# chahuja/mix-stage

Measured on AMD Instinct MI355X. Metric: train-step clips/sec (B=32, T=64, M=8), higher is better.
Workload: dtype f32; 1 GPU; Mix-StAGE GAN train step (reference D/G coin flip, seed 4321: 457 G + 510 D steps), B=32 clips per GPU, T=64, 128-mel, 104-dim pose, M=S=8, audio branch pinned; fp32 arithmetic (the reference trains in fp64, trainer.py:138; held to it at 1e-4 pose L1); global_batch=32, parallelism=dp1, hip_graphs=True, bn_sync=local

## Files before the change

### include/mixstage_aux.h

```cpp
#ifndef MIXSTAGE_AUX_H_
#define MIXSTAGE_AUX_H_

#include "mixstage.h"

#ifdef __cplusplus
extern "C" {
#endif

int ms_set_counter_buffer(int32_t* zeroed_counters, int n);

int ms_conv_block_bwd_overlap(const ms_conv_desc* d, const float* x, const float* x2, const float* w,
                              const float* gamma, const float* running_mean, const float* running_var,
                              const float* y_raw, const float* y, const float* save, const float* dy, float* dyr,
                              float* dx, float* dx2, float* dw, float* dbias, float* dgamma, float* dbeta,
                              void* workspace, size_t workspace_bytes, void* stream, void* side_stream,
                              void* side_workspace, size_t side_workspace_bytes);

int ms_timing_enable(int on);
size_t ms_timing_report(char* buf, size_t cap);

int ms_debug_set_patch_min_workgroups(int n);
int ms_debug_set_patch_tuning(int intra_split, int force_splitk);

int ms_debug_set_conv16_tile(int wm, int wn);
int ms_debug_set_conv16_ring(int nstg, int wide8);
int ms_debug_set_wgrad16_target(int workgroups);
int ms_debug_set_wgrad16_ring(int buffers);
int ms_debug_set_wgrad_target(int workgroups);
int ms_debug_set_wgrad_wave(int on);
int ms_debug_set_conv_tile(int on);
int ms_debug_set_bn_fused(int on);
int ms_debug_set_bn_fused_min_workgroups(int n);
int ms_debug_set_skip(const char* patterns);

int ms_debug_set_clip32(int on);

int ms_debug_set_clip_corun(int on);
int ms_debug_set_clip_corun_bwd(int on);

int ms_selftest_mfma(const float* A, const float* B, float* C, int K, void* stream);
int ms_probe_peak(int kind, long iters, void* a, void* b, double* work, void* stream);

#ifdef __cplusplus
}
#endif
#endif
```

### mix_stage_amd/_lib.py

```python
import ctypes
import os

_HERE = os.path.dirname(os.path.abspath(__file__))
LIB_PATH = os.path.join(_HERE, 'libmixstage_hip.so')
_ALT_LIB = os.environ.get('MS_LIB_PATH')
if _ALT_LIB:
  LIB_PATH = _ALT_LIB

c_void_p, c_int, c_float, c_size_t = ctypes.c_void_p, ctypes.c_int, ctypes.c_float, ctypes.c_size_t


class BwdOptions(ctypes.Structure):
  _fields_ = [('side_stream', ctypes.c_void_p), ('side_workspace', ctypes.c_void_p), ('side_workspace_bytes', ctypes.c_size_t),
              ('wt_prepared', ctypes.c_void_p), ('wgrad_partials', ctypes.c_void_p), ('defer_wgrad_launch', ctypes.c_int),
              ('prev_y', ctypes.c_void_p), ('prev_y_raw', ctypes.c_void_p), ('prev_save', ctypes.c_void_p), ('prev_gamma', ctypes.c_void_p),
              ('prev_dgamma', ctypes.c_void_p), ('prev_dbeta', ctypes.c_void_p), ('prev_dbias', ctypes.c_void_p), ('prev_slope', ctypes.c_float),
              ('bn_sync', ctypes.c_void_p), ('bn_sync_words', ctypes.c_int32), ('dy_is_dyr', ctypes.c_int),
              ('dx_accum', ctypes.c_void_p)]


class LossScale(ctypes.Structure):
  _fields_ = [('scale', ctypes.c_float), ('scale_dev', ctypes.c_void_p)]


# ... 126 lines not shown
    'ms_debug_set_patch_min_workgroups': (c_int, [c_int]),
    'ms_debug_set_patch_tuning': (c_int, [c_int, c_int]),
    'ms_debug_set_conv16_tile': (c_int, [c_int, c_int]),
    'ms_debug_set_conv16_ring': (c_int, [c_int, c_int]),
    'ms_debug_set_skip': (c_int, [ctypes.c_char_p]),
    'ms_debug_set_clip32': (c_int, [c_int]),
    'ms_debug_set_clip_corun': (c_int, [c_int]),
    'ms_clip_hold': (c_int, [_P]),
    'ms_clip_hold_flush': (c_int, [_P]),
    'ms_clip_hold_discard': (c_int, [_P]),
    'ms_clip_grid': (c_int, [_DESC]),
    'ms_clip_pair_ok': (c_int, [_DESC, _DESC]),
    'ms_clip_dgrad_grid': (c_int, [_DESC]),
    'ms_clip_dgrad_pair_ok': (c_int, [_DESC, _DESC]),
    'ms_debug_set_clip_corun_bwd': (c_int, [c_int]),
    'ms_debug_set_wgrad16_target': (c_int, [c_int]),
    'ms_debug_set_wgrad16_ring': (c_int, [c_int]),
    'ms_debug_set_wgrad_target': (c_int, [c_int]),
    'ms_debug_set_wgrad_wave': (c_int, [c_int]),
    'ms_debug_set_conv_tile': (c_int, [c_int]),
    'ms_set_wgrad_batched': (c_int, [c_int, c_int]),
    'ms_dgrad_fuses_prev_bn': (c_int, [_P]),
    'ms_dgrad_takes_accum': (c_int, [_P]),
    'ms_stat_pair_ok': (c_int, [_P]),
    'ms_selftest_mfma': (c_int, [_P, _P, _P, c_int, _P]),
    'ms_probe_peak': (c_int, [c_int, ctypes.c_long, _P, _P, ctypes.POINTER(ctypes.c_double), _P]),
}

_lib = None

# ... 17 lines not shown
    mode = os.environ.get('MS_PRECISION', '')
    if mode:
      if mode not in ('fp32', 'bf16x6'):
        raise MixStageLibError('MS_PRECISION=%s: expected fp32 or bf16x6' % mode)
      handle.ms_set_precision(1 if mode == 'bf16x6' else 0)
    if os.environ.get('MS_BN_FUSED'):
      handle.ms_debug_set_bn_fused(int(os.environ['MS_BN_FUSED']))
    if os.environ.get('MS_BN_FUSED_MIN_WGS'):
      handle.ms_debug_set_bn_fused_min_workgroups(int(os.environ['MS_BN_FUSED_MIN_WGS']))
    if os.environ.get('MS_CLIP32'):
      handle.ms_debug_set_clip32(int(os.environ['MS_CLIP32']))
    if os.environ.get('MS_CONV_TILE'):
      handle.ms_debug_set_conv_tile(int(os.environ['MS_CONV_TILE']))
    if os.environ.get('MS_WGRAD_WAVE'):
      handle.ms_debug_set_wgrad_wave(int(os.environ['MS_WGRAD_WAVE']))
    if os.environ.get('MS_PATCH_MIN_WGS'):
      handle.ms_debug_set_patch_min_workgroups(int(os.environ['MS_PATCH_MIN_WGS']))
    _lib = handle
  return _lib


def check(rc, what):
  if rc != 0:
    raise MixStageLibError('%s failed: %s' % (what, lib().ms_last_error().decode()))
```

### mix_stage_amd/csrc/api.hip

```cpp
#include "block_geom.h"

namespace ms {
extern int g_clip32;

static int validate(const ms_conv_desc* d, const char* who) {
  if (!d) return set_error("%s: null descriptor", who);
  if (d->B < 1 || d->Cin < 1 || d->Cout < 1 || d->groups < 1 || d->H < 1 || d->W < 1 || d->KH < 1 || d->KW < 1 ||
      d->SH < 1 || d->SW < 1 || d->PH < 0 || d->PW < 0)
    return set_error("%s: bad geometry", who);
  const int oh = (d->H + 2 * d->PH - d->KH) / d->SH + 1, ow = (d->W + 2 * d->PW - d->KW) / d->SW + 1;
  if (d->H + 2 * d->PH < d->KH || d->W + 2 * d->PW < d->KW || oh != d->OH || ow != d->OW)
    return set_error("%s: output size (%d,%d) does not match geometry (expected %d,%d)", who, d->OH, d->OW, oh, ow);
  if (d->mode < MS_BARE || d->mode > MS_BN_EVAL) return set_error("%s: bad mode %d", who, d->mode);
  if (d->in_mode < MS_IN_PLAIN || d->in_mode > MS_IN_UP2ADD) return set_error("%s: bad in_mode %d", who, d->in_mode);
  if (d->in_mode == MS_IN_UP2ADD && (d->H != 1 || d->KH != 1 || (d->W & 1)))
    return set_error("%s: UP2ADD needs a 1-D block with even W", who);
  if (dt_of(d) > DT_F16 || (d->dtype & ~(0xff | MS_DT_OUT_F32 | MS_DT_BN_FOLDED | MS_DT_STAT_PAIR))) return set_error("%s: bad dtype 0x%x", who, d->dtype);
  if (dt_of(d) == DT_F32 && (d->dtype & ~(0xff | MS_DT_STAT_PAIR))) return set_error("%s: MS_DT_OUT_F32 is a flag of the 16-bit modes", who);
  if ((d->dtype & MS_DT_STAT_PAIR) && (d->B & 1)) return set_error("%s: MS_DT_STAT_PAIR needs an even batch", who);
  const double out_elems = (double)d->B * d->groups * d->Cout * d->OH * d->OW;
  const double in_elems = (double)d->B * d->groups * d->Cin * d->H * d->W;
  const double lim = dt_of(d) == DT_F32 ? 536870912.0 : 1073741824.0;
  if (out_elems >= lim || in_elems >= lim) return set_error("%s: tensor of 2 GiB or more (%.0f elements)", who, std::max(out_elems, in_elems));
  return 0;
// ... 513 lines not shown
  float* colpart = ws_at<float>(workspace, p.ws.colpart);
  float* wt = ws_at<float>(workspace, p.ws.wt);
  float* wg_part = ws_at<float>(workspace, p.ws.wg_part);
  float* dg_part = ws_at<float>(workspace, p.ws.dg_part);
  if (defer_wgrad) wg_part = opt->wgrad_partials;
  hipStream_t ws_stream = s;
  if (side_stream && side_stream != stream && dw) {
    if (defer_wgrad) return set_error("ms_conv_block_bwd_ex: wgrad_partials and side_stream are exclusive");
    if (!opt->side_workspace || opt->side_workspace_bytes < p.ws.total)
      return set_error("ms_conv_block_bwd_overlap: side workspace too small");
    ws_stream = (hipStream_t)side_stream;
    wg_part = ws_at<float>(opt->side_workspace, p.ws.wg_part);
  }

  const float* gr = dy;
  int bias_done = 0;
  const bool have_prev = opt->prev_y != nullptr;
  if (have_prev && !(dx && g_precision == 0 && clip32_dgrad_bn_ok(d)))
    return set_error("ms_conv_block_bwd: this block's data gradient cannot carry the producer's BatchNorm backward (ms_dgrad_fuses_prev_bn)");
  if (opt->dy_is_dyr) {
    if (d->mode != MS_BN_TRAIN) return set_error("ms_conv_block_bwd: dy_is_dyr is the BN_TRAIN form");
    bias_done = 1;
  } else if (d->mode == MS_BN_TRAIN) {
    rc = launch_bn_bwd(dy, y_raw, y, save, gamma, bn_part, dyr, colpart, dbias, dgamma, dbeta, d->B, C, hw, d->slope, &bias_done, s, sg_of(d));
    gr = dyr;
  } else if (d->mode == MS_LRELU) {
    rc = launch_act_bwd(dy, y, dyr, colpart, dbias, d->B, C, hw, 1, d->slope, &bias_done, s);
    gr = dyr;
  } else if (dbias) {
    rc = launch_act_bwd(dy, nullptr, nullptr, colpart, dbias, d->B, C, hw, 0, 0.f, &bias_done, s);
  }
  if (rc) return rc;
  if (dbias && !bias_done && !opt->dy_is_dyr) {
    rc = launch_colsum_finalize(colpart, dbias, d->B, C, s);
    if (rc) return rc;
  }

  if (ws_stream != s) {
    hipEvent_t ev = fork_event();
// ... 99 lines not shown
      if (pl.splitk > 1) {
        a.part = dg_part;
        a.part_stride = dx_elems;
        a.ep = EP_DGRAD;
      }
      rc = launch_gather(a, true, up2, pl, s);
      if (rc) return rc;
      if (pl.splitk > 1) {
        rc = launch_splitk_dgrad_epilogue(dg_part, pl.splitk, dx_elems, dx, dx2, dx_elems, d->W, up2 ? 1 : 0, s);
        if (rc) return rc;
      }
    }
  }

  if (dw && p.wg_c1) {
    rc = launch_wgrad_c1(gr, x, wg_part, d->B, d->H, d->W, ws_stream);
    if (!rc && !defer_wgrad) rc = launch_reduce_splits(wg_part, dw, C * Kg, p.wg_splits, ws_stream);
    return rc;
  }
  if (dw && p.wp.ok) {
    const WgradPatchPlan& wp = p.wp;
    WgradPatchArgs q = {};
    q.dyr = gr; q.src = x; q.src2 = x2;
    q.out = wp.splits > 1 ? wg_part : dw;
    q.Cog = d->Cout; q.Cig = d->Cin; q.Kg = Kg; q.groups = d->groups; q.bcast = bcast;
    fill_src(q, plane_strides(g.one_d, d->B, g.cin_tot, d->H, d->W));
    fill_out(q, plane_strides(g.one_d, d->B, C, d->OH, d->OW));
    q.PH = g.one_d ? 0 : d->PH;
    q.PW = d->PW; q.tiles_x = wp.tiles_x; q.tiles_y = wp.tiles_y; q.n_tiles = wp.n_tiles;
    q.tiles_per_split = wp.tiles_per_split; q.splits = wp.splits;
    const double flops = 2.0 * d->Cout * q.Kg * (double)npix * d->groups;
// ... 33 lines not shown
  return clip32_fwd_pair_ok(host, guest) ? 1 : 0;
}
int ms_clip_dgrad_grid(const ms_conv_desc* d) {
  if (validate(d, "ms_clip_dgrad_grid") || dt_of(d) != DT_F32 || g_precision != 0) return 0;
  return clip32_dgrad_grid(d);
}
int ms_clip_dgrad_pair_ok(const ms_conv_desc* host, const ms_conv_desc* guest) {
  if (validate(host, "ms_clip_dgrad_pair_ok") || validate(guest, "ms_clip_dgrad_pair_ok") || dt_of(host) != DT_F32 || dt_of(guest) != DT_F32 || g_precision != 0) return 0;
  return clip32_dgrad_pair_ok(host, guest) ? 1 : 0;
}
int ms_debug_set_clip_corun(int on) {
  const int prev = g_clip_corun < 0 ? 1 : g_clip_corun;
  g_clip_corun = on ? 1 : 0;
  return prev;
}
int ms_debug_set_clip_corun_bwd(int on) {
  const int prev = g_clip_corun_bwd < 0 ? 1 : g_clip_corun_bwd;
  g_clip_corun_bwd = on ? 1 : 0;
  return prev;
}

}
```

### mix_stage_amd/csrc/conv_c1.hip

```cpp
#include <stdint.h>
#include <algorithm>
#include <stdlib.h>

#include "kernels.h"

namespace ms {

template <int CO>
__global__ __launch_bounds__(256) void conv_c1_3x3_kernel(const float* __restrict__ x, const float* __restrict__ w,
                                                          const float* __restrict__ bias, float* __restrict__ out,
                                                          const float* __restrict__ bn_g, const float* __restrict__ bn_b,
                                                          const float* __restrict__ bn_m, const float* __restrict__ bn_v,
                                                          float* __restrict__ stats, float* __restrict__ counts, int B, int H,
                                                          int W, int ep, float slope, float eps) {
  __shared__ float tile[4][CO * 65];
  const int t = threadIdx.x, lane = t & 63, wv = t >> 6;
  const int npix = B * H * W, hw = H * W;
  const int pix = blockIdx.x * 256 + t;
  const bool pv = pix < npix;
  const int b = pv ? pix / hw : 0, rem = pix - b * hw, oy = rem / W, ox = rem - oy * W;
  float xin[9];
#pragma unroll
  for (int kh = 0; kh < 3; ++kh)
#pragma unroll
// ... 178 lines not shown
          return set_error("conv_c1: cannot raise the dynamic LDS limit");                                                         \
        attr_done = 1;                                                                                                             \
      }                                                                                                                            \
      hipLaunchKernelGGL((conv_c1_3x3_v4_kernel<64, NT>), dim3(cdiv(nq, NT)), dim3(NT), lds, s, x, w, bias, out, bn_g, bn_b, bn_m,   \
                         bn_v, stats, counts, B, H, W, ep, slope, eps);                                                            \
    } while (0)
    if (nt == 64) MS_C1V(64); else if (nt == 128) MS_C1V(128); else MS_C1V(256);
#undef MS_C1V
    return check_launch("conv_c1_3x3_v4_kernel");
  }
  hipLaunchKernelGGL(conv_c1_3x3_kernel<64>, dim3(cdiv(B * H * W, 256)), dim3(256), 0, s, x, w, bias, out, bn_g, bn_b, bn_m, bn_v,
                     stats, counts, B, H, W, ep, slope, eps);
  return check_launch("conv_c1_3x3_kernel");
}

__global__ __launch_bounds__(256) void wgrad_c1_3x3_kernel(const float* __restrict__ dyr, const float* __restrict__ x,
                                                           float* __restrict__ part, int B, int H, int W, int rows_per_wg) {
  const int t = threadIdx.x, v = t & 31, cs = t >> 5;
  const int W4 = W >> 2, rows = B * H;
  const int r0 = blockIdx.x * rows_per_wg, r1 = min(rows, r0 + rows_per_wg);
  float acc[8][9];
#pragma unroll
  for (int k = 0; k < 8; ++k)
#pragma unroll
    for (int q = 0; q < 9; ++q) acc[k][q] = 0.f;
  for (int r = r0; r < r1; ++r) {
    const int b = r / H, h = r - b * H;
    for (int v0 = v; v0 < W4; v0 += 32) {
      float4 d[8];
#pragma unroll
      for (int k = 0; k < 8; ++k)
        d[k] = *reinterpret_cast<const float4*>(dyr + (((size_t)b * 64 + cs + 8 * k) * H + h) * W + 4 * v0);
      float xw[3][6];
#pragma unroll
      for (int kh = 0; kh < 3; ++kh) {
        const int hh = h + kh - 1;
        const bool rv = (unsigned)hh < (unsigned)H;
        const float* xr = x + ((size_t)b * H + (rv ? hh : h)) * W + 4 * v0;
        const float4 m = *reinterpret_cast<const float4*>(xr);
        const float lf = v0 > 0 ? xr[-1] : 0.f, rt = v0 + 1 < W4 ? xr[4] : 0.f;
        xw[kh][0] = rv ? lf : 0.f; xw[kh][1] = rv ? m.x : 0.f; xw[kh][2] = rv ? m.y : 0.f;
        xw[kh][3] = rv ? m.z : 0.f; xw[kh][4] = rv ? m.w : 0.f; xw[kh][5] = rv ? rt : 0.f;
      }
#pragma unroll
      for (int k = 0; k < 8; ++k)
#pragma unroll
        for (int kh = 0; kh < 3; ++kh)
#pragma unroll
          for (int kw = 0; kw < 3; ++kw) {
            float a = acc[k][kh * 3 + kw];
            a = fmaf(d[k].x, xw[kh][kw], a);
            a = fmaf(d[k].y, xw[kh][kw + 1], a);
            a = fmaf(d[k].z, xw[kh][kw + 2], a);
            a = fmaf(d[k].w, xw[kh][kw + 3], a);
            acc[k][kh * 3 + kw] = a;
          }
    }
  }
// ... 18 lines not shown
bool wgrad_c1_ok(int groups, int Cin, int Cout, int KH, int KW, int SH, int SW, int PH, int PW, int H, int W, int in_plain) {
  static int on = -1;
  if (on < 0) { const char* e = getenv("MS_WGRAD_C1"); on = e ? atoi(e) : 1; }
  return on && conv_c1_ok(groups, Cin, Cout, KH, KW, SH, SW, PH, PW, H, in_plain) && (W & 3) == 0;
}
int wgrad_c1_splits(int B, int H) {
  const int rows = B * H;
  return std::max(2, std::min(1024, cdiv(rows, 4)));
}
int launch_wgrad_c1(const float* dyr, const float* x, float* part, int B, int H, int W, hipStream_t s) {
  const int S = wgrad_c1_splits(B, H), rows_per_wg = cdiv(B * H, S);
  const double npix = (double)B * H * W;
  TimingScope ts(s, 2.0 * npix * 64 * 9, 4.0 * npix * 65, "wgrad_c1_3x3_kernel|conv_wgrad_c1 k3x3 Cout64 N%.0f slabs%d", npix, S);
  if (ts.skip()) return 0;
  if ((((uintptr_t)dyr | (uintptr_t)x) & 15) != 0) return set_error("wgrad_c1: unaligned tensors");
  hipLaunchKernelGGL(wgrad_c1_3x3_kernel, dim3(S), dim3(256), 0, s, dyr, x, part, B, H, W, rows_per_wg);
  return check_launch("wgrad_c1_3x3_kernel");
}

}
```

### mix_stage_amd/csrc/elementwise.hip

```cpp
#include <algorithm>

#include <stdint.h>

#include "kernels.h"
#include "conv16.h"

namespace ms {

__global__ __launch_bounds__(256) void bn_finalize_kernel(const float* __restrict__ stats,
                                                          const float* __restrict__ counts, int n_tiles, int tile_n,
                                                          int N, int C, const float* __restrict__ gamma,
                                                          const float* __restrict__ beta, float* running_mean,
                                                          float* running_var, float* __restrict__ save, float eps,
                                                          float momentum) {
  prefetch_kernargs<128>();
  __shared__ double red[4];
  const int c = blockIdx.x, t = threadIdx.x;
  double s = 0.0;
  for (int i = t; i < n_tiles; i += 256) s += (double)stats[((size_t)i * C + c) * 2];
  s = wave_sum_d(s);
  if ((t & 63) == 0) red[t >> 6] = s;
  __syncthreads();
  const double mean = (red[0] + red[1] + red[2] + red[3]) / (double)N;
  __syncthreads();
// ... 325 lines not shown
  s3 = block_sum_256(s3, red);
  if (t == 0) {
    partial[((size_t)c * gridDim.y + ch) * 2] = s1;
    partial[((size_t)c * gridDim.y + ch) * 2 + 1] = s2;
    xsum[(size_t)c * gridDim.y + ch] = s3;
  }
}

__global__ __launch_bounds__(256) void bn_bwd_apply4_kernel(const float* __restrict__ dy, const float* __restrict__ y_raw,
                                                            const float* __restrict__ save, const float* __restrict__ gamma,
                                                            const float* __restrict__ partial, float* __restrict__ dyr,
                                                            const float* __restrict__ xsum, float* dbias, float* dgamma, float* dbeta,
                                                            int B, int C, int HW, int b_per_chunk, float slope) {
  prefetch_kernargs<128>();
  const int c = blockIdx.x, ch = blockIdx.y, t = threadIdx.x, nchunk = gridDim.y;
  float s1 = 0.f, s2 = 0.f, s3 = 0.f;
  for (int k = 0; k < nchunk; ++k) {
    s1 += partial[((size_t)c * nchunk + k) * 2];
    s2 += partial[((size_t)c * nchunk + k) * 2 + 1];
    s3 += xsum[(size_t)c * nchunk + k];
  }
  const float invN = 1.0f / (float)((size_t)B * HW);
  const float mean = save[c], invstd = save[C + c], sc = save[2 * C + c], sh = save[3 * C + c];
  const float gi = gamma[c] * invstd, m1 = s1 * invN, m2 = s2 * invN;
  const int b0 = ch * b_per_chunk, nb = min(b_per_chunk, B - b0);
  const int HW4 = HW >> 2, nv = nb * HW4;
  const FastDiv fd(HW4, nv + 1024);
  for (int e0 = t; e0 < nv; e0 += 1024) {
    float4 yr[4], g[4];
    size_t off[4];
#pragma unroll
    for (int u = 0; u < 4; ++u) {
      const int e = min(e0 + 256 * u, nv - 1);
      const int b = fd.div(e), p4 = e - b * HW4;
      off[u] = ((size_t)(b0 + b) * C + c) * HW + 4 * p4;
      yr[u] = *reinterpret_cast<const float4*>(y_raw + off[u]);
      g[u] = *reinterpret_cast<const float4*>(dy + off[u]);
    }
#pragma unroll
    for (int u = 0; u < 4; ++u) {
      if (e0 + 256 * u < nv) {
        const float a[4] = {yr[u].x, yr[u].y, yr[u].z, yr[u].w}, d[4] = {g[u].x, g[u].y, g[u].z, g[u].w};
        float o[4];
#pragma unroll
        for (int j = 0; j < 4; ++j) {
          const float z = fmaf(a[j], sc, sh);
          const float dz = d[j] * (z > 0.f ? 1.f : slope);
          const float xh = (a[j] - mean) * invstd;
          o[j] = gi * (dz - m1 - xh * m2);
        }
        *reinterpret_cast<float4*>(dyr + off[u]) = float4{o[0], o[1], o[2], o[3]};
      }
    }
  }
  if (t == 0 && ch == 0) {
    if (dgamma) { dgamma[c] = s2; dbeta[c] = s1; }
    if (dbias) dbias[c] = -gi * m2 * s3;
  }
}

template <int NE>
__global__ __launch_bounds__(256) void bn_bwd_fused_kernel(const float* __restrict__ dy, const float* __restrict__ y_raw,
                                                           const float* __restrict__ y, const float* __restrict__ save,
                                                           const float* __restrict__ gamma,
                                                           float* __restrict__ dyr, float* dbias, float* dgamma, float* dbeta,
                                                           int B, int C, int HW, float slope, int sg) {
  prefetch_kernargs<128>();
  const FastDiv fdHW(HW, B * HW);
  __shared__ float red[4];
  const int c = blockIdx.x, t = threadIdx.x;
  const int n = B * HW;
  float tot_cs = 0.f, tot_s1 = 0.f, tot_s2 = 0.f;
// ... 232 lines not shown
    const float r = (float)Tout / (float)Tin;
    const int d_lo = t == 0 ? 0 : max(0, (int)floorf(((float)t - 0.5f) * r - 0.5f) - 1);
    const int d_hi = t == Tin - 1 ? Tout - 1 : min(Tout - 1, (int)ceilf(((float)t + 1.5f) * r - 0.5f) + 1);
    for (int d = d_lo; d <= d_hi; ++d) {
      int t0, t1;
      float lt;
      lerp_coords(d, Tin, Tout, t0, t1, lt);
      float wt = 0.f;
      if (t == t0) wt += 1.f - lt;
      if (t == t1) wt += lt;
      if (wt != 0.f) acc += wt * dy[(size_t)bc * Tout + d];
    }
    acc *= wf;
  }
  dx[i] = acc;
}

#define MIX_TT 64
__global__ __launch_bounds__(256) void softmax_mix_fwd_kernel(const float* __restrict__ z, const float* __restrict__ score,
                                                              float* __restrict__ soft, float* __restrict__ out, int M,
                                                              int P, int T, int FC) {
  extern __shared__ float sm[];
  float* wsm = sm;
  float* tile = sm + (size_t)M * MIX_TT;
  const int b = blockIdx.y, t0 = blockIdx.x * MIX_TT, t = threadIdx.x, lane = t & 63, w = t >> 6;
  const int f_beg = blockIdx.z * FC, nf = min(FC, P - f_beg);
  const int tt = t0 + lane;
  const bool tv = tt < T;
  if (w == 0) {
    float mx = -INFINITY;
// ... 654 lines not shown
  hipLaunchKernelGGL(bn_apply_kernel, dim3(blocks), dim3(256), 0, s, y_raw, y, save, C, HW, total, slope);
  return check_launch("bn_apply_kernel");
}

int bwd_chunks(int B, int C, int* b_per_chunk) {
  int want = C >= 1024 ? 1 : (1024 + C - 1) / C;
  if (want > B) want = B;
  if (want < 1) want = 1;
  const int bpc = (B + want - 1) / want;
  *b_per_chunk = bpc;
  return (B + bpc - 1) / bpc;
}

int launch_bn_bwd(const float* dy, const float* y_raw, const float* y, const float* save, const float* gamma, float* partial, float* dyr,
                  float* colpart, float* dbias, float* dgamma, float* dbeta, int B, int C, int HW, float slope, int* fused,
                  hipStream_t s, int sg) {
  *fused = 0;
  if (sg > 1) B /= sg;
  const long n = (long)B * HW;
  if (sg > 1 && n > BN_BWD32_FUSED_MAX) return set_error("bn_bwd: statistics groups need the one-launch form (%ld values per channel)", n);
  if (n <= BN_BWD32_FUSED_MAX) {
    const bool vec4 = (HW & 3) == 0 && (((uintptr_t)dy | (uintptr_t)y_raw | (uintptr_t)y | (uintptr_t)dyr) & 15) == 0;
    const int ne = vec4 ? (n <= 1024 ? 1 : n <= 2048 ? 2 : 4) : (n <= 256 * 4 ? 4 : n <= 256 * 8 ? 8 : 16);
    TimingScope ts(s, 0, 12.0 * sg * B * C * HW, "bn_bwd_fused%s<%d> C%d HW%d B%d%s", vec4 ? "4" : "", ne, C, HW, B * sg, sg > 1 ? " pair" : "");
    if (ts.skip()) { *fused = 1; return 0; }
    if (vec4 && n <= 1024)
      hipLaunchKernelGGL(bn_bwd_fused4_kernel<1>, dim3(C), dim3(256), 0, s, dy, y_raw, y, save, gamma, dyr, dbias, dgamma, dbeta, B, C, HW, slope, sg);
    else if (vec4 && n <= 2048)
      hipLaunchKernelGGL(bn_bwd_fused4_kernel<2>, dim3(C), dim3(256), 0, s, dy, y_raw, y, save, gamma, dyr, dbias, dgamma, dbeta, B, C, HW, slope, sg);
    else if (vec4)
      hipLaunchKernelGGL(bn_bwd_fused4_kernel<4>, dim3(C), dim3(256), 0, s, dy, y_raw, y, save, gamma, dyr, dbias, dgamma, dbeta, B, C, HW, slope, sg);
    else if (n <= 256 * 4)
      hipLaunchKernelGGL(bn_bwd_fused_kernel<4>, dim3(C), dim3(256), 0, s, dy, y_raw, y, save, gamma, dyr, dbias, dgamma, dbeta, B, C, HW, slope, sg);
    else if (n <= 256 * 8)
      hipLaunchKernelGGL(bn_bwd_fused_kernel<8>, dim3(C), dim3(256), 0, s, dy, y_raw, y, save, gamma, dyr, dbias, dgamma, dbeta, B, C, HW, slope, sg);
    else
      hipLaunchKernelGGL(bn_bwd_fused_kernel<16>, dim3(C), dim3(256), 0, s, dy, y_raw, y, save, gamma, dyr, dbias, dgamma, dbeta, B, C, HW, slope, sg);
    *fused = 1;
    return check_launch("bn_bwd_fused_kernel");
  }
  int bpc;
  const int nchunk = bwd_chunks(B, C, &bpc);
  const bool vec = (HW & 3) == 0 && (((uintptr_t)dy | (uintptr_t)y_raw | (uintptr_t)dyr) & 15) == 0;
  TimingScope ts(s, 0, 20.0 * B * C * HW, "bn_bwd(%s) C%d HW%d B%d", vec ? "reduce4+apply4" : "reduce+apply", C, HW, B);
  if (ts.skip()) return 0;
  if (vec) hipLaunchKernelGGL(bn_bwd_reduce4_kernel, dim3(C, nchunk), dim3(256), 0, s, dy, y_raw, save, partial, colpart, B, C, HW, bpc, slope);
  else hipLaunchKernelGGL(bn_bwd_reduce_kernel, dim3(C, nchunk), dim3(256), 0, s, dy, y_raw, save, partial, B, C, HW, bpc, slope);
  int rc = check_launch("bn_bwd_reduce_kernel");
  if (rc) return rc;
  if (vec) {
    hipLaunchKernelGGL(bn_bwd_apply4_kernel, dim3(C, nchunk), dim3(256), 0, s, dy, y_raw, save, gamma, partial, dyr, colpart, dbias,
                       dgamma, dbeta, B, C, HW, bpc, slope);
    *fused = 1;
  } else {
    hipLaunchKernelGGL(bn_bwd_apply_kernel, dim3(C, nchunk), dim3(256), 0, s, dy, y_raw, save, gamma, partial, dyr, colpart,
                       dgamma, dbeta, B, C, HW, bpc, slope);
  }
  return check_launch("bn_bwd_apply_kernel");
}

int launch_act_bwd(const float* dy, const float* y, float* dyr, float* colpart, float* dbias, int B, int C, int HW, int mode, float slope,
                   int* fused, hipStream_t s) {
  *fused = 0;
  const long nn = (long)B * HW;
// ... 37 lines not shown

extern "C" {

int ms_lerp_time_fwd(const float* x, float* y, int B, int C, int Tin, int F, int Tout, void* stream) {
  TimingScope ts((hipStream_t)stream, 0, 0, "ew|ew_lerp_time_fwd");
  if (ts.skip()) return 0;
  const int n = B * C * Tout;
  hipLaunchKernelGGL(lerp_time_fwd_kernel, dim3(cdiv(n, 256)), dim3(256), 0, (hipStream_t)stream, x, y, B * C, Tin, F, Tout);
  return check_launch("lerp_time_fwd_kernel");
}

int ms_lerp_time_bwd(const float* dy, float* dx, int B, int C, int Tin, int F, int Tout, void* stream) {
  TimingScope ts((hipStream_t)stream, 0, 0, "ew|ew_lerp_time_bwd");
  if (ts.skip()) return 0;
  const int n = B * C * Tin * F;
  hipLaunchKernelGGL(lerp_time_bwd_kernel, dim3(cdiv(n, 256)), dim3(256), 0, (hipStream_t)stream, dy, dx, B * C, Tin, F, Tout);
  return check_launch("lerp_time_bwd_kernel");
}

int ms_softmax_mix_fwd(const float* z, const float* score, float* soft, float* out, int B, int M, int P, int T, void* stream) {
  TimingScope ts((hipStream_t)stream, 0, 0, "ew|ew_softmax_mix_fwd");
  if (ts.skip()) return 0;
  const int tiles = cdiv(T, MIX_TT) * B;
  int nch = std::max(1, std::min(P, 512 / std::max(1, tiles)));
  const int fc = cdiv(P, nch);
  nch = cdiv(P, fc);
  const size_t lds = ((size_t)M * MIX_TT + (size_t)MIX_TT * (fc + 1)) * sizeof(float);
  if (lds > 160 * 1024) return set_error("ms_softmax_mix_fwd: M=%d P=%d needs %zu B of LDS", M, P, lds);
  hipLaunchKernelGGL(softmax_mix_fwd_kernel, dim3(cdiv(T, MIX_TT), B, nch), dim3(256), lds, (hipStream_t)stream, z, score, soft,
                     out, M, P, T, fc);
// ... 402 lines not shown
```

### mix_stage_amd/csrc/kernels.h

```cpp
#pragma once
#include "common.h"

namespace ms {

enum { EP_BARE = 0, EP_LRELU = 1, EP_BN_EVAL = 2, EP_RAW_STATS = 3, EP_DGRAD = 4, EP_DGRAD_UP2 = 5, EP_BN_FUSED = 6, EP_DGRAD_BN = 7, EP_DGRAD_ACC = 8 };

struct GatherArgs {
  const float* A;
  const float* src;
  const float* src2;
  float* out;
  float* out2;
  const float* bias;
  const float* bn_g;
  const float* bn_b;
  const float* bn_m;
  const float* bn_v;
  float* stats;
  int Mg, Kg, groups, Kc, src_ctotal, SRCH, SRCW, OUTH, OUTW, Npix;
  int KH, KW, SH, SW, PH, PW;
  int bcast, a_vec, ep;
  int batch;
  int splitk, k_per_split;
  float* part;
// ... 62 lines not shown
struct PatchPlan { int ok, tm, tw, tiles_y, tiles_x, n_tiles, splitk, chunks_per_split, tn, wm, ksi, p6, tile; };
PatchPlan plan_patch(int nd, int Mg, int groups, int Kc, int KH, int KW, int SH, int SW, int B, int OH, int OW, int zmul = 1, int in_w = 0);
extern int g_conv_tile;
bool conv_tile_shape_ok(int KH, int KW, int S);
int launch_tile(const PatchArgs& a, const PatchPlan& pl, int KH, int KW, int S, double flops, double bytes, hipStream_t s);
int patch_chunk_channels(int KH, int KW);
bool patch_dgrad_direct_ok(const float* w, int Cin_g, int KH, int KW, int SH, int SW, bool up2_or_bcast);
int launch_patch(const PatchArgs& a, const PatchPlan& pl, int KH, int KW, int S, bool up2, double flops, double bytes,
                 hipStream_t s);

bool conv_c1_ok(int groups, int Cin, int Cout, int KH, int KW, int SH, int SW, int PH, int PW, int H, int in_plain);
int conv_c1_tiles(int B, int H, int W);
bool wgrad_c1_ok(int groups, int Cin, int Cout, int KH, int KW, int SH, int SW, int PH, int PW, int H, int W, int in_plain);
int wgrad_c1_splits(int B, int H);
int launch_wgrad_c1(const float* dyr, const float* x, float* part, int B, int H, int W, hipStream_t s);
int launch_conv_c1(const float* x, const float* w, const float* bias, float* out, const float* bn_g, const float* bn_b,
                   const float* bn_m, const float* bn_v, float* stats, float* counts, int B, int H, int W, int ep, float slope,
                   float eps, hipStream_t s);
extern int g_patch_intra;
extern int g_precision;
bool patch6_supported(int KH, int KW, int S);
int patch6_row_elems(int Kc, int KH, int KW);
int launch_split_weights(const float* w, unsigned short* planes, int rows, int Kc, int KH, int KW, hipStream_t s);
struct SplitJob {
  const float* w;
  unsigned short* planes;
  int rows, Kc, KHW, CK, row_elems, block_end;
};
enum { SPLIT_BATCH_MAX = 64 };
struct SplitBatch { int n; SplitJob job[SPLIT_BATCH_MAX]; };
// ... 129 lines not shown
struct TransposeBatch { int n; TransposeJob job[TRANSPOSE_BATCH_MAX]; };
int launch_transpose_weight_multi(TransposeBatch& tb, hipStream_t s);
int launch_transpose_weight(const float* w, float* wt, int groups, int Cog, int Cig, int KH, int KW, int SH, int SW,
                            int PH, int PW, int flip, hipStream_t s);
size_t dgrad_weight_elems(int groups, int Cog, int Cig, int KH, int KW, int SH, int SW);
int launch_bn_finalize(const float* stats, const float* counts, int n_tiles, int tile_n, int N, int C, const float* gamma,
                       const float* beta, float* rm, float* rv, float* save, float eps, float momentum, hipStream_t s);
int launch_bn_apply(const float* y_raw, float* y, const float* save, int C, int HW, size_t total, float slope, hipStream_t s);
int launch_bn_finalize_apply(const float* stats, const float* counts, int n_tiles, int tile_n, int N, int C, const float* gamma,
                             const float* beta, float* rm, float* rv, float* save, float eps, float momentum, const float* y_raw,
                             float* y, int B, int HW, float slope, hipStream_t s);
int bwd_chunks(int B, int C, int* b_per_chunk);
constexpr int BN_BWD32_FUSED_MAX = 256 * 16;
int launch_bn_bwd(const float* dy, const float* y_raw, const float* y, const float* save, const float* gamma, float* partial, float* dyr,
                  float* colpart, float* dbias, float* dgamma, float* dbeta, int B, int C, int HW, float slope, int* fused,
                  hipStream_t s, int sg = 1);
int launch_act_bwd(const float* dy, const float* y, float* dyr, float* colpart, float* dbias, int B, int C, int HW, int mode, float slope, int* fused,
                   hipStream_t s);
int launch_colsum_finalize(const float* colpart, float* out, int B, int C, hipStream_t s);
int launch_adam_seg(float* p, const float* g, float* m, float* v, size_t n, const int32_t* step_state, const int32_t* seg_of_chunk,
                    const float* seg_scratch, float beta1, float beta2, float eps, hipStream_t s);

__device__ inline float adam_seg_step_size(float lr, float beta1, double t) { return (float)((double)lr / (1.0 - pow((double)beta1, t))); }
__device__ inline float adam_seg_bc2(float beta2, double t) { return (float)sqrt(1.0 - pow((double)beta2, t)); }
__device__ inline float adam_clip_coef(float max_norm, float n) {
  const float coef = max_norm / (n + 1e-6f);
  return coef > 1.f ? 1.f : coef;
}
__device__ inline bool adam_norm_finite(float n) { return fabsf(n) <= 3.0e38f; }
__device__ inline bool adam_lr_bad(float lr) { return !(lr > 0.f && lr <= 3.0e38f); }
__device__ inline void adam_flag_step(int32_t* state, bool bad) {
// ... 42 lines not shown
```

Measured before the change: 11460 clips/s.

## Fuse BN backward apply into first-layer wgrad kernel and add row-tiled lerp backward

New measurement: 11520 clips/s (median of 6 runs). About the same (+0.6%).

```diff
diff --git a/include/mixstage_aux.h b/include/mixstage_aux.h
--- a/include/mixstage_aux.h
+++ b/include/mixstage_aux.h
@@ -37,6 +37,7 @@
 
 int ms_debug_set_clip_corun(int on);
 int ms_debug_set_clip_corun_bwd(int on);
+int ms_debug_set_c1_bwd_fused(int on);
 
 int ms_selftest_mfma(const float* A, const float* B, float* C, int K, void* stream);
 int ms_probe_peak(int kind, long iters, void* a, void* b, double* work, void* stream);
diff --git a/mix_stage_amd/_lib.py b/mix_stage_amd/_lib.py
--- a/mix_stage_amd/_lib.py
+++ b/mix_stage_amd/_lib.py
@@ -164,6 +164,7 @@
     'ms_clip_dgrad_grid': (c_int, [_DESC]),
     'ms_clip_dgrad_pair_ok': (c_int, [_DESC, _DESC]),
     'ms_debug_set_clip_corun_bwd': (c_int, [c_int]),
+    'ms_debug_set_c1_bwd_fused': (c_int, [c_int]),
     'ms_debug_set_wgrad16_target': (c_int, [c_int]),
     'ms_debug_set_wgrad16_ring': (c_int, [c_int]),
     'ms_debug_set_wgrad_target': (c_int, [c_int]),
@@ -211,6 +212,8 @@
       handle.ms_debug_set_conv_tile(int(os.environ['MS_CONV_TILE']))
     if os.environ.get('MS_WGRAD_WAVE'):
       handle.ms_debug_set_wgrad_wave(int(os.environ['MS_WGRAD_WAVE']))
+    if os.environ.get('MS_C1_BWD_FUSED') and hasattr(handle, 'ms_debug_set_c1_bwd_fused'):
+      handle.ms_debug_set_c1_bwd_fused(int(os.environ['MS_C1_BWD_FUSED']))
     if os.environ.get('MS_PATCH_MIN_WGS'):
       handle.ms_debug_set_patch_min_workgroups(int(os.environ['MS_PATCH_MIN_WGS']))
     _lib = handle
diff --git a/mix_stage_amd/csrc/api.hip b/mix_stage_amd/csrc/api.hip
--- a/mix_stage_amd/csrc/api.hip
+++ b/mix_stage_amd/csrc/api.hip
@@ -551,7 +551,7 @@
   }
 
   const float* gr = dy;
-  int bias_done = 0;
+  int bias_done = 0, c1_bn = 0;
   const bool have_prev = opt->prev_y != nullptr;
   if (have_prev && !(dx && g_precision == 0 && clip32_dgrad_bn_ok(d)))
     return set_error("ms_conv_block_bwd: this block's data gradient cannot carry the producer's BatchNorm backward (ms_dgrad_fuses_prev_bn)");
@@ -559,7 +559,9 @@
     if (d->mode != MS_BN_TRAIN) return set_error("ms_conv_block_bwd: dy_is_dyr is the BN_TRAIN form");
     bias_done = 1;
   } else if (d->mode == MS_BN_TRAIN) {
-    rc = launch_bn_bwd(dy, y_raw, y, save, gamma, bn_part, dyr, colpart, dbias, dgamma, dbeta, d->B, C, hw, d->slope, &bias_done, s, sg_of(d));
+    const bool c1_ask = g_c1_bwd_fused && p.wg_c1 && dw && !dx && ws_stream == s && sg_of(d) == 1;
+    rc = launch_bn_bwd(dy, y_raw, y, save, gamma, bn_part, dyr, colpart, dbias, dgamma, dbeta, d->B, C, hw, d->slope, &bias_done, s, sg_of(d),
+                       c1_ask ? &c1_bn : nullptr);
     gr = dyr;
   } else if (d->mode == MS_LRELU) {
     rc = launch_act_bwd(dy, y, dyr, colpart, dbias, d->B, C, hw, 1, d->slope, &bias_done, s);
@@ -689,7 +691,8 @@
   }
 
   if (dw && p.wg_c1) {
-    rc = launch_wgrad_c1(gr, x, wg_part, d->B, d->H, d->W, ws_stream);
+    rc = c1_bn ? launch_wgrad_c1_bn(dy, y_raw, save, gamma, bn_part, colpart, dbias, dgamma, dbeta, d->slope, x, wg_part, d->B, d->H, d->W, ws_stream)
+               : launch_wgrad_c1(gr, x, wg_part, d->B, d->H, d->W, ws_stream);
     if (!rc && !defer_wgrad) rc = launch_reduce_splits(wg_part, dw, C * Kg, p.wg_splits, ws_stream);
     return rc;
   }
@@ -753,6 +756,11 @@
   g_clip_corun = on ? 1 : 0;
   return prev;
 }
+int ms_debug_set_c1_bwd_fused(int on) {
+  const int prev = g_c1_bwd_fused;
+  g_c1_bwd_fused = on ? 1 : 0;
+  return prev;
+}
 int ms_debug_set_clip_corun_bwd(int on) {
   const int prev = g_clip_corun_bwd < 0 ? 1 : g_clip_corun_bwd;
   g_clip_corun_bwd = on ? 1 : 0;
diff --git a/mix_stage_amd/csrc/conv_c1.hip b/mix_stage_amd/csrc/conv_c1.hip
--- a/mix_stage_amd/csrc/conv_c1.hip
+++ b/mix_stage_amd/csrc/conv_c1.hip
@@ -216,11 +216,30 @@
   return check_launch("conv_c1_3x3_kernel");
 }
 
-__global__ __launch_bounds__(256) void wgrad_c1_3x3_kernel(const float* __restrict__ dyr, const float* __restrict__ x,
-                                                           float* __restrict__ part, int B, int H, int W, int rows_per_wg) {
+struct C1BnBwd {
+  const float* y_raw; const float* save; const float* gamma; const float* partial; const float* xsum;
+  float* dbias; float* dgamma; float* dbeta;
+  int nchunk;
+  float slope, invN;
+};
+template <bool BN>
+__global__ __launch_bounds__(256, 2) void wgrad_c1_3x3_kernel(const float* __restrict__ dyr, const float* __restrict__ x,
+                                                           float* __restrict__ part, int B, int H, int W, int rows_per_wg, C1BnBwd bn) {
   const int t = threadIdx.x, v = t & 31, cs = t >> 5;
   const int W4 = W >> 2, rows = B * H;
   const int r0 = blockIdx.x * rows_per_wg, r1 = min(rows, r0 + rows_per_wg);
+  __shared__ __attribute__((aligned(16))) float bnk[BN ? 64 : 1][8];
+  if constexpr (BN) {
+    if (t < 64) {
+      const BnBwdChannel k = bn_bwd_channel(bn.partial, bn.xsum, bn.save, bn.gamma, t, 64, bn.nchunk, bn.invN);
+      bnk[t][0] = k.mean; bnk[t][1] = k.invstd; bnk[t][2] = k.sc; bnk[t][3] = k.sh; bnk[t][4] = k.gi; bnk[t][5] = k.m1; bnk[t][6] = k.m2;
+      if (blockIdx.x == 0) {
+        if (bn.dgamma) { bn.dgamma[t] = k.s2; bn.dbeta[t] = k.s1; }
+        if (bn.dbias) bn.dbias[t] = bn_bwd_dbias(k);
+      }
+    }
+    __syncthreads();
+  }
   float acc[8][9];
 #pragma unroll
   for (int k = 0; k < 8; ++k)
@@ -229,10 +248,13 @@
   for (int r = r0; r < r1; ++r) {
     const int b = r / H, h = r - b * H;
     for (int v0 = v; v0 < W4; v0 += 32) {
-      float4 d[8];
-#pragma unroll
-      for (int k = 0; k < 8; ++k)
-        d[k] = *reinterpret_cast<const float4*>(dyr + (((size_t)b * 64 + cs + 8 * k) * H + h) * W + 4 * v0);
+      float4 d[8], yr[BN ? 8 : 1];
+#pragma unroll
+      for (int k = 0; k < 8; ++k) {
+        const size_t off = (((size_t)b * 64 + cs + 8 * k) * H + h) * W + 4 * v0;
+        d[k] = *reinterpret_cast<const float4*>(dyr + off);
+        if constexpr (BN) yr[k] = *reinterpret_cast<const float4*>(bn.y_raw + off);
+      }
       float xw[3][6];
 #pragma unroll
       for (int kh = 0; kh < 3; ++kh) {
@@ -244,6 +266,19 @@
         xw[kh][0] = rv ? lf : 0.f; xw[kh][1] = rv ? m.x : 0.f; xw[kh][2] = rv ? m.y : 0.f;
         xw[kh][3] = rv ? m.z : 0.f; xw[kh][4] = rv ? m.w : 0.f; xw[kh][5] = rv ? rt : 0.f;
       }
+      if constexpr (BN) {
+        asm volatile("" ::: "memory");
+#pragma unroll
+        for (int k = 0; k < 8; ++k) {
+          const float4 c0 = *reinterpret_cast<const float4*>(&bnk[cs + 8 * k][0]), c1 = *reinterpret_cast<const float4*>(&bnk[cs + 8 * k][4]);
+          BnBwdChannel kc;
+          kc.mean = c0.x; kc.invstd = c0.y; kc.sc = c0.z; kc.sh = c0.w; kc.gi = c1.x; kc.m1 = c1.y; kc.m2 = c1.z;
+          d[k].x = bn_bwd_dyr(yr[k].x, d[k].x, kc, bn.slope);
+          d[k].y = bn_bwd_dyr(yr[k].y, d[k].y, kc, bn.slope);
+          d[k].z = bn_bwd_dyr(yr[k].z, d[k].z, kc, bn.slope);
+          d[k].w = bn_bwd_dyr(yr[k].w, d[k].w, kc, bn.slope);
+        }
+      }
 #pragma unroll
       for (int k = 0; k < 8; ++k)
 #pragma unroll
@@ -292,8 +327,23 @@
   TimingScope ts(s, 2.0 * npix * 64 * 9, 4.0 * npix * 65, "wgrad_c1_3x3_kernel|conv_wgrad_c1 k3x3 Cout64 N%.0f slabs%d", npix, S);
   if (ts.skip()) return 0;
   if ((((uintptr_t)dyr | (uintptr_t)x) & 15) != 0) return set_error("wgrad_c1: unaligned tensors");
-  hipLaunchKernelGGL(wgrad_c1_3x3_kernel, dim3(S), dim3(256), 0, s, dyr, x, part, B, H, W, rows_per_wg);
+  hipLaunchKernelGGL(wgrad_c1_3x3_kernel<false>, dim3(S), dim3(256), 0, s, dyr, x, part, B, H, W, rows_per_wg, C1BnBwd{});
   return check_launch("wgrad_c1_3x3_kernel");
 }
 
-}
+int g_c1_bwd_fused = 1;
+int launch_wgrad_c1_bn(const float* dy, const float* y_raw, const float* save, const float* gamma, const float* partial, const float* xsum,
+                       float* dbias, float* dgamma, float* dbeta, float slope, const float* x, float* part, int B, int H, int W,
+                       hipStream_t s) {
+  const int S = wgrad_c1_splits(B, H), rows_per_wg = cdiv(B * H, S);
+  const double npix = (double)B * H * W;
+  TimingScope ts(s, 2.0 * npix * 64 * 9, 4.0 * npix * 129, "wgrad_c1_3x3_kernel|conv_wgrad_c1 k3x3 Cout64 N%.0f slabs%d +bnbwd", npix, S);
+  if (ts.skip()) return 0;
+  if ((((uintptr_t)dy | (uintptr_t)y_raw | (uintptr_t)x) & 15) != 0) return set_error("wgrad_c1: unaligned tensors");
+  int bpc;
+  C1BnBwd bn = {y_raw, save, gamma, partial, xsum, dbias, dgamma, dbeta, bwd_chunks(B, 64, &bpc), slope, 1.0f / (float)((size_t)B * H * W)};
+  hipLaunchKernelGGL(wgrad_c1_3x3_kernel<true>, dim3(S), dim3(256), 0, s, dy, x, part, B, H, W, rows_per_wg, bn);
+  return check_launch("wgrad_c1_3x3_kernel");
+}
+
+}
diff --git a/mix_stage_amd/csrc/elementwise.hip b/mix_stage_amd/csrc/elementwise.hip
--- a/mix_stage_amd/csrc/elementwise.hip
+++ b/mix_stage_amd/csrc/elementwise.hip
@@ -363,15 +363,7 @@
                                                             int B, int C, int HW, int b_per_chunk, float slope) {
   prefetch_kernargs<128>();
   const int c = blockIdx.x, ch = blockIdx.y, t = threadIdx.x, nchunk = gridDim.y;
-  float s1 = 0.f, s2 = 0.f, s3 = 0.f;
-  for (int k = 0; k < nchunk; ++k) {
-    s1 += partial[((size_t)c * nchunk + k) * 2];
-    s2 += partial[((size_t)c * nchunk + k) * 2 + 1];
-    s3 += xsum[(size_t)c * nchunk + k];
-  }
-  const float invN = 1.0f / (float)((size_t)B * HW);
-  const float mean = save[c], invstd = save[C + c], sc = save[2 * C + c], sh = save[3 * C + c];
-  const float gi = gamma[c] * invstd, m1 = s1 * invN, m2 = s2 * invN;
+  const BnBwdChannel k = bn_bwd_channel(partial, xsum, save, gamma, c, C, nchunk, 1.0f / (float)((size_t)B * HW));
   const int b0 = ch * b_per_chunk, nb = min(b_per_chunk, B - b0);
   const int HW4 = HW >> 2, nv = nb * HW4;
   const FastDiv fd(HW4, nv + 1024);
@@ -392,19 +384,14 @@
         const float a[4] = {yr[u].x, yr[u].y, yr[u].z, yr[u].w}, d[4] = {g[u].x, g[u].y, g[u].z, g[u].w};
         float o[4];
 #pragma unroll
-        for (int j = 0; j < 4; ++j) {
-          const float z = fmaf(a[j], sc, sh);
-          const float dz = d[j] * (z > 0.f ? 1.f : slope);
-          const float xh = (a[j] - mean) * invstd;
-          o[j] = gi * (dz - m1 - xh * m2);
-        }
+        for (int j = 0; j < 4; ++j) o[j] = bn_bwd_dyr(a[j], d[j], k, slope);
         *reinterpret_cast<float4*>(dyr + off[u]) = float4{o[0], o[1], o[2], o[3]};
       }
     }
   }
   if (t == 0 && ch == 0) {
-    if (dgamma) { dgamma[c] = s2; dbeta[c] = s1; }
-    if (dbias) dbias[c] = -gi * m2 * s3;
+    if (dgamma) { dgamma[c] = k.s2; dbeta[c] = k.s1; }
+    if (dbias) dbias[c] = bn_bwd_dbias(k);
   }
 }
 
@@ -667,6 +654,87 @@
     acc *= wf;
   }
   dx[i] = acc;
+}
+
+constexpr int LERP_ROWS_MAX_T = 1024;
+constexpr int LERP_ROWS_DY = 4096;
+__global__ __launch_bounds__(256) void lerp_time_bwd_rows_kernel(const float* __restrict__ dy, float* __restrict__ dx, int BC, int Tin,
+                                                                 int F, int Tout, int R, int dy_vec, int dx_vec) {
+  __shared__ float4 sco[LERP_ROWS_MAX_T];
+  __shared__ float sdy[LERP_ROWS_DY];
+  __shared__ float sacc[LERP_ROWS_MAX_T];
+  const int tid = threadIdx.x;
+  const int row0 = blockIdx.x * R, nr = min(R, BC - row0);
+  const int ld = Tout + 1;
+  const float* src = dy + (size_t)row0 * Tout;
+  const int n = nr * Tout, n4 = dy_vec ? n >> 2 : 0;
+  const FastDiv fdT(Tout, n + 4096);
+  float4 q[4];
+  if (n4 > 0) {
+#pragma unroll
+    for (int u = 0; u < 4; ++u) q[u] = *reinterpret_cast<const float4*>(src + 4 * (size_t)min(tid + 256 * u, n4 - 1));
+  }
+  for (int d = tid; d < Tout; d += 256) {
+    int t0, t1;
+    float lt;
+    lerp_coords(d, Tin, Tout, t0, t1, lt);
+    sco[d] = float4{__int_as_float(t0), __int_as_float(t1), 1.f - lt, lt};
+  }
+  for (int i0 = tid; i0 < n4; i0 += 1024) {
+    if (i0 != tid) {
+#pragma unroll
+      for (int u = 0; u < 4; ++u) q[u] = *reinterpret_cast<const float4*>(src + 4 * (size_t)min(i0 + 256 * u, n4 - 1));
+    }
+#pragma unroll
+    for (int u = 0; u < 4; ++u) {
+      const int i = i0 + 256 * u;
+      if (i < n4) {
+        const int r = fdT.div(4 * i);
+        float* o = sdy + r * ld + (4 * i - r * Tout);
+        o[0] = q[u].x; o[1] = q[u].y; o[2] = q[u].z; o[3] = q[u].w;
+      }
+    }
+  }
+  for (int i = 4 * n4 + tid; i < n; i += 256) {
+    const int r = fdT.div(i);
+    sdy[r * ld + (i - r * Tout)] = src[i];
+  }
+  __syncthreads();
+  const FastDiv fdTin(Tin, nr * Tin + 256);
+  const float rr = (float)Tout / (float)Tin;
+  for (int it = tid; it < nr * Tin; it += 256) {
+    const int r = fdTin.div(it), t = it - r * Tin;
+    const int d_lo = t == 0 ? 0 : max(0, (int)floorf(((float)t - 0.5f) * rr - 0.5f) - 1);
+    const int d_hi = t == Tin - 1 ? Tout - 1 : min(Tout - 1, (int)ceilf(((float)t + 1.5f) * rr - 0.5f) + 1);
+    const float* row = sdy + r * ld;
+    float acc = 0.f;
+    for (int d = d_lo; d <= d_hi; ++d) {
+      const float4 c = sco[d];
+      float wt = 0.f;
+      if (t == __float_as_int(c.x)) wt += c.z;
+      if (t == __float_as_int(c.y)) wt += c.w;
+      const float g = row[d];
+      if (wt != 0.f) acc += wt * g;
+    }
+    sacc[it] = acc;
+  }
+  __syncthreads();
+  int f0, f1;
+  float lf;
+  lerp_coords(0, F, 1, f0, f1, lf);
+  float* dst = dx + (size_t)row0 * Tin * F;
+  const int m = nr * Tin * F, m4 = dx_vec ? m >> 2 : 0;
+  const FastDiv fdF(F, m + 4);
+  auto value = [&](int e) {
+    const int rt = fdF.div(e), f = e - rt * F;
+    float wf = 0.f;
+    if (f == f0) wf += 1.f - lf;
+    if (f == f1) wf += lf;
+    return wf != 0.f ? sacc[rt] * wf : 0.f;
+  };
+  for (int i = tid; i < m4; i += 256)
+    *reinterpret_cast<float4*>(dst + 4 * (size_t)i) = float4{value(4 * i), value(4 * i + 1), value(4 * i + 2), value(4 * i + 3)};
+  for (int e = 4 * m4 + tid; e < m; e += 256) dst[e] = value(e);
 }
 
 #define MIX_TT 64
@@ -1351,8 +1419,10 @@
 
 int launch_bn_bwd(const float* dy, const float* y_raw, const float* y, const float* save, const float* gamma, float* partial, float* dyr,
                   float* colpart, float* dbias, float* dgamma, float* dbeta, int B, int C, int HW, float slope, int* fused,
-                  hipStream_t s, int sg) {
+                  hipStream_t s, int sg, int* defer_apply) {
   *fused = 0;
+  const bool may_defer = defer_apply != nullptr;
+  if (defer_apply) *defer_apply = 0;
   if (sg > 1) B /= sg;
   const long n = (long)B * HW;
   if (sg > 1 && n > BN_BWD32_FUSED_MAX) return set_error("bn_bwd: statistics groups need the one-launch form (%ld values per channel)", n);
@@ -1379,12 +1449,19 @@
   int bpc;
   const int nchunk = bwd_chunks(B, C, &bpc);
   const bool vec = (HW & 3) == 0 && (((uintptr_t)dy | (uintptr_t)y_raw | (uintptr_t)dyr) & 15) == 0;
-  TimingScope ts(s, 0, 20.0 * B * C * HW, "bn_bwd(%s) C%d HW%d B%d", vec ? "reduce4+apply4" : "reduce+apply", C, HW, B);
+  const bool defer = may_defer && vec;
+  TimingScope ts(s, 0, (defer ? 8.0 : 20.0) * B * C * HW, "bn_bwd(%s) C%d HW%d B%d%s", vec ? "reduce4+apply4" : "reduce+apply", C, HW, B,
+                 defer ? " apply-in-wgrad" : "");
   if (ts.skip()) return 0;
   if (vec) hipLaunchKernelGGL(bn_bwd_reduce4_kernel, dim3(C, nchunk), dim3(256), 0, s, dy, y_raw, save, partial, colpart, B, C, HW, bpc, slope);
   else hipLaunchKernelGGL(bn_bwd_reduce_kernel, dim3(C, nchunk), dim3(256), 0, s, dy, y_raw, save, partial, B, C, HW, bpc, slope);
   int rc = check_launch("bn_bwd_reduce_kernel");
   if (rc) return rc;
+  if (defer) {
+    *defer_apply = 1;
+    *fused = 1;
+    return 0;
+  }
   if (vec) {
     hipLaunchKernelGGL(bn_bwd_apply4_kernel, dim3(C, nchunk), dim3(256), 0, s, dy, y_raw, save, gamma, partial, dyr, colpart, dbias,
                        dgamma, dbeta, B, C, HW, bpc, slope);
@@ -1452,6 +1529,13 @@
   TimingScope ts((hipStream_t)stream, 0, 0, "ew|ew_lerp_time_bwd");
   if (ts.skip()) return 0;
   const int n = B * C * Tin * F;
+  if (Tin <= LERP_ROWS_MAX_T && Tout <= LERP_ROWS_MAX_T) {
+    const int R = std::max(1, std::min(std::min(256 / Tin, LERP_ROWS_DY / (Tout + 1)), B * C));
+    const int dy_vec = (Tout & 3) == 0 && ((uintptr_t)dy & 15) == 0, dx_vec = ((R * Tin * F) & 3) == 0 && ((uintptr_t)dx & 15) == 0;
+    hipLaunchKernelGGL(lerp_time_bwd_rows_kernel, dim3(cdiv(B * C, R)), dim3(256), 0, (hipStream_t)stream, dy, dx, B * C, Tin, F, Tout, R,
+                       dy_vec, dx_vec);
+    return check_launch("lerp_time_bwd_rows_kernel");
+  }
   hipLaunchKernelGGL(lerp_time_bwd_kernel, dim3(cdiv(n, 256)), dim3(256), 0, (hipStream_t)stream, dy, dx, B * C, Tin, F, Tout);
   return check_launch("lerp_time_bwd_kernel");
 }
diff --git a/mix_stage_amd/csrc/kernels.h b/mix_stage_amd/csrc/kernels.h
--- a/mix_stage_amd/csrc/kernels.h
+++ b/mix_stage_amd/csrc/kernels.h
@@ -100,6 +100,10 @@
 bool wgrad_c1_ok(int groups, int Cin, int Cout, int KH, int KW, int SH, int SW, int PH, int PW, int H, int W, int in_plain);
 int wgrad_c1_splits(int B, int H);
 int launch_wgrad_c1(const float* dyr, const float* x, float* part, int B, int H, int W, hipStream_t s);
+extern int g_c1_bwd_fused;
+int launch_wgrad_c1_bn(const float* dy, const float* y_raw, const float* save, const float* gamma, const float* partial, const float* xsum,
+                       float* dbias, float* dgamma, float* dbeta, float slope, const float* x, float* part, int B, int H, int W,
+                       hipStream_t s);
 int launch_conv_c1(const float* x, const float* w, const float* bias, float* out, const float* bn_g, const float* bn_b,
                    const float* bn_m, const float* bn_v, float* stats, float* counts, int B, int H, int W, int ep, float slope,
                    float eps, hipStream_t s);
@@ -259,7 +263,32 @@
 constexpr int BN_BWD32_FUSED_MAX = 256 * 16;
 int launch_bn_bwd(const float* dy, const float* y_raw, const float* y, const float* save, const float* gamma, float* partial, float* dyr,
                   float* colpart, float* dbias, float* dgamma, float* dbeta, int B, int C, int HW, float slope, int* fused,
-                  hipStream_t s, int sg = 1);
+                  hipStream_t s, int sg = 1, int* defer_apply = nullptr);
+
+struct BnBwdChannel {
+  float mean, invstd, sc, sh, gi, m1, m2, s1, s2, s3;
+};
+__device__ __forceinline__ BnBwdChannel bn_bwd_channel(const float* __restrict__ partial, const float* __restrict__ xsum,
+                                                       const float* __restrict__ save, const float* __restrict__ gamma, int c, int C,
+                                                       int nchunk, float invN) {
+  BnBwdChannel k;
+  float s1 = 0.f, s2 = 0.f, s3 = 0.f;
+  for (int j = 0; j < nchunk; ++j) {
+    s1 += partial[((size_t)c * nchunk + j) * 2];
+    s2 += partial[((size_t)c * nchunk + j) * 2 + 1];
+    s3 += xsum[(size_t)c * nchunk + j];
+  }
+  k.s1 = s1; k.s2 = s2; k.s3 = s3;
+  k.mean = save[c]; k.invstd = save[C + c]; k.sc = save[2 * C + c]; k.sh = save[3 * C + c];
+  k.gi = gamma[c] * k.invstd; k.m1 = s1 * invN; k.m2 = s2 * invN;
+  return k;
+}
+__device__ __forceinline__ float bn_bwd_dyr(float yr, float g, const BnBwdChannel& k, float slope) {
+  const float z = fmaf(yr, k.sc, k.sh);
+  const float xh = (yr - k.mean) * k.invstd;
+  return k.gi * fmaf(-k.m2, xh, fmaf(g, z > 0.f ? 1.f : slope, -k.m1));
+}
+__device__ __forceinline__ float bn_bwd_dbias(const BnBwdChannel& k) { return -k.gi * k.m2 * k.s3; }
 int launch_act_bwd(const float* dy, const float* y, float* dyr, float* colpart, float* dbias, int B, int C, int HW, int mode, float slope, int* fused,
                    hipStream_t s);
 int launch_colsum_finalize(const float* colpart, float* out, int B, int C, hipStream_t s);
```
